# vineety/sparse_matrix_mult

Hardware: AMD Instinct MI355X
Metric: output nnz/sec, CSR x CSR -> CSR SpGEMM (first-touch order, float64) (higher is better)
Workload: dtype f64

## Files before the change

### sparse_matrix_mult_amd/csrc/smm_api.hip

```cpp
#include "smm_kernels.hpp"
#include "smm_slab.hpp"
#include "smm_ring.hpp"
#include "smm_triple_sparse.hpp"
#include "smm_masked.hpp"
#include "smm_spmm.hpp"
#include "smm_kron.hpp"
#include "smm_cg.hpp"
#include "smm_slq.hpp"
#include "smm_sddmm.hpp"
#include "smm_taper.hpp"
#include "smm_interp.hpp"
#include "../../include/smm_hip.h"

#include <sys/mman.h>
#include <unistd.h>

#include <algorithm>
#include <atomic>
#include <cmath>
#include <condition_variable>
#include <cstdarg>
#include <cstdio>
#include <cstring>
#include <map>
// ... 82 lines not shown
    hipEvent_t cg_ev[2] = {nullptr, nullptr};
    int exact_checked = 0;
    int check = 0;
    int inject_alloc_nth = 0;
    bool inject_alloc_hard = false;
    int64_t alloc_retries = 0;
    unsigned *d_flags = nullptr;
    unsigned *d_err = nullptr;
    std::recursive_mutex mu;
};
#define CTX_LOCK(c) std::lock_guard<std::recursive_mutex> ctx_lock_((c)->mu)

static void pool_flush(smm_ctx *c)
{
    for (auto &b : c->pool) (void)hipFree(b.p);
    c->pool.clear();
}
static hipError_t dev_malloc(smm_ctx *c, void **p, size_t bytes)
{
    bool fail_first = false, fail_both = false;
    if (c->inject_alloc_nth > 0 && --c->inject_alloc_nth == 0) { fail_first = true; fail_both = c->inject_alloc_hard; }
    hipError_t e = fail_first ? hipErrorOutOfMemory : hipMalloc(p, bytes);
    if (e == hipSuccess) return e;
    (void)hipGetLastError();
    pool_flush(c);
    ++c->alloc_retries;
    e = fail_both ? hipErrorOutOfMemory : hipMalloc(p, bytes);
    if (e != hipSuccess) { (void)hipGetLastError(); *p = nullptr; }
    return e;
}

static int pool_alloc(smm_ctx *c, size_t bytes, void **out)
{
    if (bytes == 0) bytes = 16;
    bytes = (bytes + 255) & ~(size_t)255;
    int best = -1;
    for (int i = 0; i < (int)c->pool.size(); ++i)
        if (c->pool[i].bytes >= bytes && c->pool[i].bytes <= bytes + bytes / 4 + (1 << 20) &&
            (best < 0 || c->pool[i].bytes < c->pool[best].bytes))
            best = i;
    if (best >= 0) {
        *out = c->pool[best].p;
        c->live[*out] = c->pool[best].bytes;
        c->pool.erase(c->pool.begin() + best);
        return SMM_OK;
    }
    void *p = nullptr;
    hipError_t e = dev_malloc(c, &p, bytes);
    if (e != hipSuccess) return fail(SMM_ERR_ALLOC, "hipMalloc of %zu bytes failed: %s", bytes, hipGetErrorString(e));
    c->live[p] = bytes;
    *out = p;
    return SMM_OK;
}
static void pool_free(smm_ctx *c, void *p)
{
    if (!p) return;
    auto it = c->live.find(p);
    if (it == c->live.end()) return;
    c->pool.push_back({p, it->second});
    c->live.erase(it);
}
template <typename T> static int pool_get(smm_ctx *c, size_t count, T **out)
{
    void *p = nullptr;
    int rc = pool_alloc(c, count * sizeof(T), &p);
    *out = (T *)p;
    return rc;
}

template <typename T> struct PoolBuf {
    smm_ctx *c;
    T *p = nullptr;
    explicit PoolBuf(smm_ctx *ctx) : c(ctx) {}
    PoolBuf(PoolBuf &&o) noexcept : c(o.c), p(o.release()) {}
    PoolBuf &operator=(PoolBuf &&o) noexcept { if (this != &o) { reset(); c = o.c; p = o.release(); } return *this; }
    ~PoolBuf() { reset(); }
    int alloc(size_t count) { reset(); return pool_get(c, count, &p); }
    void reset() { pool_free(c, p); p = nullptr; }
    T *release() { T *q = p; p = nullptr; return q; }
    operator T *() const { return p; }
};
template <typename T> struct DevBuf {
    T *p = nullptr;
    int64_t bytes = 0;
    DevBuf() = default;
    DevBuf(DevBuf &&o) noexcept : p(o.p), bytes(o.bytes) { o.p = nullptr; o.bytes = 0; }
    DevBuf &operator=(DevBuf &&o) noexcept { if (this != &o) { reset(); std::swap(p, o.p); std::swap(bytes, o.bytes); } return *this; }
    ~DevBuf() { reset(); }
    hipError_t alloc(smm_ctx *c, size_t count)
    {
        reset();
        const hipError_t e = dev_malloc(c, (void **)&p, count * sizeof(T));
        if (e == hipSuccess) bytes = (int64_t)(count * sizeof(T));
        return e;
    }
    void reset() { if (p) (void)hipFree(p); p = nullptr; bytes = 0; }
    operator T *() const { return p; }
};
template <auto Destroy> struct Destroyer {
    template <typename T> void operator()(T *x) const { Destroy(x); }
};

struct LaunchTimer {
    smm_ctx *c; const char *name; hipEvent_t t0 = nullptr, t1 = nullptr;
    LaunchTimer(smm_ctx *ctx, const char *n) : c(ctx), name(n)
    {
// ... 917 lines not shown
    if (lds > 64 * 1024)
        HIPCHK(hipFuncSetAttribute((const void *)kern, hipFuncAttributeMaxDynamicSharedMemorySize, (int)lds));
    int64_t grid = (int64_t)args.m * args.nct;
    if (grid > 0x7fffffff) return fail(SMM_ERR_INVALID, "too many (row, tile) units for one launch");
    args.unit_counter = nullptr; args.n_units = (unsigned)grid;
    const bool persist = c->numeric_persist == 2 || (c->numeric_persist == 1 && OUT == OUT_SPARSE);
    if (persist && grid > c->n_cu) {
        const int64_t per_cu = std::max<int64_t>(1, std::min<int64_t>(32 / NW, (int64_t)(160 * 1024) / (int64_t)(lds + 64)));
        args.unit_counter = (unsigned *)((char *)c->d_flags + 220);
        HIPCHK(hipMemsetAsync(args.unit_counter, 0, sizeof(unsigned), c->stream));
        grid = std::min<int64_t>(grid, per_cu * c->n_cu);
    }
#ifdef SMM_STAMPS
    PoolBuf<unsigned long long> d_st(c);
    CHK(d_st.alloc(4));
    (void)hipMemsetAsync(d_st, 0, 32, c->stream);
    args.stamps = d_st;
#endif
    LAUNCH(c, SCR ? "smm_emit" : OUT == OUT_SPARSE ? "smm_numeric" : "smm_numeric_dense", kern, grid, NW * 64, lds, args);
    hipError_t e = hipGetLastError();
#ifdef SMM_STAMPS
    {
        unsigned long long h[4];
        (void)hipMemcpyAsync(h, d_st, 32, hipMemcpyDeviceToHost, c->stream);
        (void)hipStreamSynchronize(c->stream);
        const double tot = (double)(h[0] + h[1] + h[2]);
        fprintf(stderr, "[SMM_STAMPS] units=%lld NW=%d wc=%d nct=%d exact=%d  init %.1f%%  accumulate %.1f%%  epilogue %.1f%%  (sum %.3g cycles)\n",
                (long long)grid, NW, args.wc, args.nct, (int)EXACT, 100 * h[0] / tot, 100 * h[1] / tot, 100 * h[2] / tot, tot);
        d_st.reset();
    }
#endif
    if (e != hipSuccess) return fail(SMM_ERR_HIP, "smm_numeric launch: %s", hipGetErrorString(e));
    return SMM_OK;
}
template <int OUT>
static int launch_numeric(smm_ctx *c, NumericArgs &args, bool sym, int nw, bool exact)
{
    if (args.m <= 0) return SMM_OK;
    args.dummy_idx = (const int *)((const char *)c->d_flags + 64);
    args.dummy_val = (const double *)((const char *)c->d_flags + 128);
    args.err = c->d_err;
#define SMM_CASE(S, N, X) \
    if (sym == S && nw == N && exact == X) return launch_numeric_t<OUT, S, N, X>(c, args);
    SMM_CASE(false, 1, true) SMM_CASE(true, 1, true) SMM_CASE(false, 2, true) SMM_CASE(true, 2, true)
    SMM_CASE(false, 4, true) SMM_CASE(true, 4, true) SMM_CASE(false, 8, true) SMM_CASE(true, 8, true)
    SMM_CASE(false, 16, true) SMM_CASE(true, 16, true)
    SMM_CASE(false, 4, false) SMM_CASE(true, 4, false) SMM_CASE(false, 8, false) SMM_CASE(true, 8, false)
    SMM_CASE(false, 16, false) SMM_CASE(true, 16, false)
#undef SMM_CASE
    return fail(SMM_ERR_INVALID, "unsupported numeric configuration");
}

constexpr size_t LIST_SLACK = (size_t)1 << 17;
#ifndef SMM_CCS_UNROLL
#define SMM_CCS_UNROLL 8
#endif
using ccs_kernel_t = decltype(&smm_symbolic_ccs<false, SMM_CCS_UNROLL>);
static ccs_kernel_t ccs_kernel(bool sym, bool dr, bool batch)
{
#define CCS_K(S, D, B) smm_symbolic_ccs<S, SMM_CCS_UNROLL, D, B>
    if (batch) return dr ? (sym ? CCS_K(true, true, 16) : CCS_K(false, true, 16)) : (sym ? CCS_K(true, false, 16) : CCS_K(false, false, 16));
    return dr ? (sym ? CCS_K(true, true, 1) : CCS_K(false, true, 1)) : (sym ? CCS_K(true, false, 1) : CCS_K(false, false, 1));
#undef CCS_K
}
struct SlabGeom { int ws, n_slabs, rw; };
constexpr int SLAB_NW = 8;
struct smm_plan {
    smm_ctx *ctx = nullptr;
    smm_csr *a = nullptr, *b = nullptr;
    int flags = 0;
    int64_t row_offset = 0;
    int64_t m = 0, ncols = 0, nnz = 0;
    bool b_sorted = true;
    Geom g{};
    int64_t *d_ub_off = nullptr;
    void *d_tmp = nullptr;
    bool list16 = false;
    unsigned *d_P = nullptr;
    unsigned *d_runs = nullptr;
    int2 *d_tail = nullptr;
    int n_slabs = 1, tps = 0, ws = 0;
    int *d_scnt = nullptr;
    unsigned *d_dst0 = nullptr;
    uint2 *d_runs2 = nullptr;
    unsigned char *d_tflag = nullptr;
    const int *seg = nullptr;
    const short *loc = nullptr;
    smm_csr::PackView pack{0, 0, nullptr, nullptr, 0, 0};
    bool use_slab = false;
    SlabGeom sg{};
    smm_csr::SlabView slab{0, 0, nullptr, nullptr, nullptr};
    int *d_rowcnt = nullptr;
    int64_t total_cap = 0;
    int *d_lists = nullptr;
    int n_bin[8] = {0, 0, 0, 0, 0, 0, 0, 0};
    int64_t *d_cptr = nullptr;
};

extern "C" void smm_plan_destroy(smm_plan *p)
{
    if (!p) return;
    smm_ctx *c = p->ctx;
    CTX_LOCK(c);
    (void)hipSetDevice(c->device);
    (void)hipStreamSynchronize(c->stream);
    pool_free(c, p->d_ub_off); pool_free(c, p->d_tmp); pool_free(c, p->d_P); pool_free(c, p->d_runs);
// ... 576 lines not shown
static int sym_slab_walk(smm_ctx *c, smm_plan *p, SymRows &r)
{
    r.slists.reset();
    r.prod.reset();
    smm_csr *a = p->a, *b = p->b;
    const int64_t m = p->m;
    const int ws_cap = c->sym_max_ws > 0 ? c->sym_max_ws : CCS_MAX_WS;
    int tps = std::max(1, std::min(8, ws_cap / p->g.wc));
    if (c->sym_max_ws == 0)
        while (tps > 1 && (160 * 1024) / ((((tps * p->g.wc + 31) / 32) + WAVE) * 4) < 28) --tps;
    p->tps = tps; p->ws = tps * p->g.wc; p->n_slabs = (p->g.nct + tps - 1) / tps;
    p->list16 = true;
    const int ns = p->n_slabs;
    smm_csr::CcsView cc{};
    CHK(ensure_ccs(c, b, p->ws, ns, &cc));
    const int *sseg = nullptr;
    CHK(ensure_seg(c, b, tiles_geom(ns, p->ws), &sseg));
    PoolBuf<int64_t> ubs(c);
    CHK(ubs.alloc((size_t)ns * m));
    pool_free(c, p->d_ub_off); p->d_ub_off = nullptr;
    CHK(pool_get(c, (size_t)ns * m + 1, &p->d_ub_off));
    LAUNCH(c, "smm_row_work", smm_ccs_row_work, (int)std::min<int64_t>((m + 3) / 4, 16384), 256, 0, (int)m, ns, p->ws, (int)p->ncols,
           (int)b->rows, p->row_offset, (p->flags & SMM_SYMMETRIC) ? 1 : 0, a->ptr, a->idx, sseg, ubs.p);
    CHK(scan_launch<int64_t>(c, (int64_t)ns * m, ubs, p->d_ub_off));
    HIPCHK(hipMemcpyAsync(&p->total_cap, p->d_ub_off + (int64_t)ns * m, sizeof(int64_t), hipMemcpyDeviceToHost, c->stream));
    HIPCHK(hipStreamSynchronize(c->stream));
    ubs.reset();
    CHK(pool_alloc(c, ((size_t)std::max<int64_t>(p->total_cap, 1) + LIST_SLACK) * 2, &p->d_tmp));
    CHK(pool_get(c, (size_t)a->nnz * ns, &p->d_P));
    CHK(pool_get(c, (size_t)ns * m, &p->d_scnt));
    CHK(pool_get(c, (size_t)m, &p->d_rowcnt));
    int *d_unitctr = (int *)((char *)c->d_flags + 208);
    HIPCHK(hipMemsetAsync(d_unitctr, 0, sizeof(int), c->stream));
    if ((int64_t)ns * m >= INT32_MAX) return fail(SMM_ERR_INVALID, "too many (slab, row) units");
    CHK(launch_ccs(c, p, cc, (int64_t)ns * m, ns, nullptr, nullptr, p->d_scnt, d_unitctr));
    LAUNCH(c, "smm_slab_rowcnt", smm_slab_rowcnt, std::min<int64_t>((m + 255) / 256, 4096), 256, 0, (int)m, ns, (const int *)p->d_scnt,
           p->d_rowcnt);
    CHK(scan_launch<int>(c, m, p->d_rowcnt, p->d_cptr));
    HIPCHK(hipMemcpyAsync(&p->nnz, p->d_cptr + m, sizeof(int64_t), hipMemcpyDeviceToHost, c->stream));
    HIPCHK(hipStreamSynchronize(c->stream));
    LAUNCH_CHECK();
    if (p->nnz > 0) CHK(bin_c_rows(c, p, BinSpec{2, {0, 0, 0, 0, 0, 0}, 3, 4}, nullptr));
    if (p->n_bin[2] > 0) {
        if (p->flags & SMM_EXACT) {
            CHK(ensure_seg(c, b, p->g, &p->seg));
            CHK(ensure_loc(c, b, p->g, &p->loc));
        } else {
            CHK(ensure_pack(c, b, p->g, PACK_FMT_16, &p->pack));
        }
        CHK(pool_get(c, (size_t)a->nnz, &p->d_dst0));
        CHK(pool_get(c, (size_t)a->nnz * p->g.nct, &p->d_runs2));
        CHK(pool_get(c, (size_t)m * p->g.nct, &p->d_tflag));
        const int nd = p->n_bin[2];
        LAUNCH(c, "smm_runs", smm_runs_slab, std::min<int64_t>((nd + 3) / 4, 65536), 256, 0, nd, (int)m, ns, tps, p->g.nct, p->g.wc,
               (int64_t)a->nnz, (const int *)(p->d_lists + 2 * m), a->ptr, (const int64_t *)p->d_ub_off, (const int *)p->d_scnt,
               (const unsigned *)p->d_P, (const unsigned short *)p->d_tmp, p->d_dst0, p->d_runs2, p->d_tflag, c->d_err);
        LAUNCH_CHECK();
    }
    return SMM_OK;
}

static int sym_row_walk(smm_ctx *c, smm_plan *p, SymRows &r)
{
    smm_csr *a = p->a, *b = p->b;
    const int64_t m = p->m;
    const bool sym = (p->flags & SMM_SYMMETRIC) != 0;
    const bool safe = r.safe;
    p->list16 = c->narrow_idx && p->ncols < 65535 && b->cols < 65535;
    if (p->list16) CHK(ensure_idx16(c, b));
    p->total_cap = r.total_ub;
    CHK(pool_alloc(c, ((size_t)std::max<int64_t>(r.total_ub, 1) + std::max<size_t>(LIST_SLACK, (size_t)p->ncols)) * (p->list16 ? 2 : 4),
                   &p->d_tmp));
    CHK(pool_get(c, (size_t)a->nnz, &p->d_P));
    CHK(pool_get(c, (size_t)m, &p->d_rowcnt));
    if (r.binned) HIPCHK(hipMemsetAsync(p->d_rowcnt, 0, (size_t)m * sizeof(int), c->stream));
    int *d_rowctr = (int *)((char *)c->d_flags + 288);
    HIPCHK(hipMemsetAsync(d_rowctr, 0, 8 * sizeof(int), c->stream));
    int *d_scounts = (int *)((char *)c->d_flags + 256);
    const int *d_slists = r.slists;
    for (int tc = 0; tc < 2; ++tc) {
        const int bin = tc == 0 ? SB_TINY : SB_TINY2;
        const int nt = r.sbin[bin];
        if (nt == 0) continue;
        const int per_wg = tc == 0 ? 16 : 8;
        const int tgrid = (int)std::min<int64_t>(((int64_t)nt + per_wg - 1) / per_wg, (int64_t)c->n_cu * 32);
        const int *rows3 = d_slists + (size_t)bin * m;
#define TINY_CASE(S, IT, G)                                                                                                      \
        LAUNCH(c, "smm_symbolic_tiny", (smm_symbolic_tiny<S, IT, G>), tgrid, 256, 0, nt, rows3, p->row_offset, a->ptr, a->idx,     \
               b->ptr, b->idx, (const int64_t *)p->d_ub_off, (IT *)p->d_tmp, p->d_P, p->d_rowcnt, c->d_err);
#define TINY_G_CASE(S, IT) if (tc == 0) { TINY_CASE(S, IT, TINY_G) } else { TINY_CASE(S, IT, TINY_G2) }
        if (p->list16) { if (sym) { TINY_G_CASE(true, unsigned short) } else { TINY_G_CASE(false, unsigned short) } }
        else           { if (sym) { TINY_G_CASE(true, int) } else { TINY_G_CASE(false, int) } }
#undef TINY_G_CASE
#undef TINY_CASE
        LAUNCH_CHECK();
    }
    for (int cls = 0; cls < NHC; ++cls) {
        if (r.hmax1 == 0 || r.sbin[cls] == 0) continue;
        const int hs = HS[cls];
        const int hgrid = (int)std::min<int64_t>((r.sbin[cls] + 3) / 4, (int64_t)c->n_cu * 16);
        if (sym) CHK((launch_symbolic_t<true, false, MARK_LDS_HASH>(c, p, hs, nullptr, hgrid, 4, d_slists + (size_t)cls * m, d_scounts + cls, d_rowctr + cls)));
        else     CHK((launch_symbolic_t<false, false, MARK_LDS_HASH>(c, p, hs, nullptr, hgrid, 4, d_slists + (size_t)cls * m, d_scounts + cls, d_rowctr + cls)));
    }
    const int bm_words = (int)((p->ncols + 31) / 32);
    const size_t bm_bytes = (size_t)(bm_words + 1) * sizeof(unsigned);
    const bool ldsbm = bm_bytes <= 128 * 1024;
// ... 6 lines not shown
    PoolBuf<unsigned> gbm(c);
    const bool use_ccs = c->sym_ccs && p->list16 && !safe && p->ncols <= CCS_MAX_WS && nbm > 0;
    if (use_ccs) {
        smm_csr::CcsView cc{};
        CHK(ensure_ccs(c, b, (int)p->ncols, 1, &cc));
        CHK(launch_ccs(c, p, cc, nbm, 1, bm_rows, bm_count, p->d_rowcnt, d_rowctr + SB_REST));
    } else if (nbm > 0) {
        int sgrid = (int)std::min<int64_t>((nbm + wpb - 1) / wpb, (int64_t)c->n_cu * 8 * (4 / wpb));
        if (!ldsbm) CHK(gbm.alloc((size_t)sgrid * wpb * (bm_words + 1)));
        const int mark = ldsbm ? MARK_LDS_BITMAP : MARK_GLOBAL_BITMAP;
        const int rbatch = nbm >= (int64_t)64 * sgrid * wpb && nbm < INT32_MAX - (1 << 24) ? 16 : 1;
#define SYM_CASE(S, F, L) if (sym == S && safe == F && mark == L && !deep) CHK((launch_symbolic_t<S, F, L>(c, p, bm_words, gbm, sgrid, wpb, bm_rows, bm_count, d_rowctr + SB_REST, rbatch)));
        SYM_CASE(false, false, MARK_LDS_BITMAP) SYM_CASE(false, true, MARK_LDS_BITMAP) SYM_CASE(true, false, MARK_LDS_BITMAP)
        SYM_CASE(true, true, MARK_LDS_BITMAP) SYM_CASE(false, false, MARK_GLOBAL_BITMAP) SYM_CASE(false, true, MARK_GLOBAL_BITMAP)
        SYM_CASE(true, false, MARK_GLOBAL_BITMAP) SYM_CASE(true, true, MARK_GLOBAL_BITMAP)
#define SYM_DEEP(S, L) if (sym == S && mark == L && deep) CHK((launch_symbolic_t<S, false, L, 32>(c, p, bm_words, gbm, sgrid, wpb, bm_rows, bm_count, d_rowctr + SB_REST, rbatch)));
        SYM_DEEP(false, MARK_LDS_BITMAP) SYM_DEEP(true, MARK_LDS_BITMAP) SYM_DEEP(false, MARK_GLOBAL_BITMAP) SYM_DEEP(true, MARK_GLOBAL_BITMAP)
#undef SYM_DEEP
#undef SYM_CASE
    }
    CHK(scan_launch<int>(c, m, p->d_rowcnt, p->d_cptr));
    HIPCHK(hipMemcpyAsync(&p->nnz, p->d_cptr + m, sizeof(int64_t), hipMemcpyDeviceToHost, c->stream));
    HIPCHK(hipStreamSynchronize(c->stream));
    LAUNCH_CHECK();
    gbm.reset();
    r.slists.reset();
    return SMM_OK;
}

static int sym_runs(smm_ctx *c, smm_plan *p, SymRows &r)
{
    smm_csr *a = p->a, *b = p->b;
    const int64_t m = p->m;
    if (p->nnz > 0) CHK(bin_c_rows(c, p, BinSpec{2, {c->hash_small, c->hash_medium, 0, 0, 0, 0}, 3, 4}, r.prod));
    r.prod.reset();
    if (!p->b_sorted || p->n_bin[2] == 0) return SMM_OK;
    const double est_products = (double)a->nnz * ((double)b->nnz / (double)std::max<int64_t>(b->rows, 1)) * ((double)p->n_bin[2] / (double)m);
    p->use_slab = slab_geometry(c, b, p->ncols, &p->sg) &&
                  slab_pays(c, a, p->sg, (double)p->n_bin[2] * (double)p->ncols, est_products, (double)p->nnz,
                            (double)b->nnz / (double)std::max<int64_t>(b->rows, 1), (double)p->ncols);
    if (p->use_slab) CHK(ensure_slab(c, b, p->sg, &p->slab));
    if (p->use_slab && c->slab_mode == 2) {  }
    else if (p->flags & SMM_EXACT) {
        CHK(ensure_seg(c, b, p->g, &p->seg));
        CHK(ensure_loc(c, b, p->g, &p->loc));
    } else {
        CHK(ensure_pack(c, b, p->g, p->use_slab ? PACK_FMT_16 : PACK_FMT_12, &p->pack));
    }
    CHK(pool_get(c, (size_t)a->nnz * (p->g.nct + 1), &p->d_runs));
    CHK(pool_get(c, (size_t)m, &p->d_tail));
    const int nd = p->n_bin[2];
    const int rgrid = (int)std::min<int64_t>((nd + 3) / 4, 65536);
    const int tail_min = (p->flags & SMM_EXACT) ? TAIL_MIN_EXACT : TAIL_MIN_DEFAULT;
    if (p->list16)
        LAUNCH(c, "smm_runs", smm_runs<unsigned short>, rgrid, 256, 0, nd, p->g.nct, p->g.wc, (const int *)(p->d_lists + 2 * m), a->ptr,
               p->d_ub_off, p->d_rowcnt, p->d_P, (const unsigned short *)p->d_tmp, p->d_runs, p->d_tail, c->d_err, tail_min);
    else
        LAUNCH(c, "smm_runs", smm_runs<int>, rgrid, 256, 0, nd, p->g.nct, p->g.wc, (const int *)(p->d_lists + 2 * m), a->ptr,
               p->d_ub_off, p->d_rowcnt, p->d_P, (const int *)p->d_tmp, p->d_runs, p->d_tail, c->d_err, tail_min);
    LAUNCH_CHECK();
    return SMM_OK;
}

extern "C" int smm_spgemm_symbolic(smm_ctx *c, smm_csr *a, smm_csr *b, int flags, int64_t a_row_offset,
                                   smm_plan **plan, int64_t *nnz_out)
{
    if (!plan) return fail(SMM_ERR_INVALID, "plan is NULL");
    *plan = nullptr;
    if (!c) return fail(SMM_ERR_INVALID, "ctx is NULL");
    CTX_LOCK(c);
    CHK(check_pair(c, a, b));
    if (a_row_offset < 0) return fail(SMM_ERR_INVALID, "negative a_row_offset");
    CHK(exact_guard(c, flags));
    PlanPtr p(new smm_plan());
    p->ctx = c; p->a = a; p->b = b; p->flags = flags; p->row_offset = a_row_offset;
    p->m = a->rows; p->ncols = b->cols;
    p->b_sorted = !(b->vflags & CSR_UNSORTED);
    p->g = make_geom(c, p->ncols, b, (flags & SMM_EXACT) != 0);
    CHK(pool_get(c, (size_t)p->m + 1, &p->d_cptr));
    if (p->m == 0 || a->nnz == 0 || b->nnz == 0 || p->ncols == 0) {
        HIPCHK(hipMemsetAsync(p->d_cptr, 0, (p->m + 1) * sizeof(int64_t), c->stream));
    } else {
        SymRows r(c);
        CHK(sym_row_work(c, p.get(), r));
        if (use_slab_walk(c, p.get(), r)) {
            CHK(sym_slab_walk(c, p.get(), r));
        } else {
            CHK(sym_row_walk(c, p.get(), r));
            CHK(sym_runs(c, p.get(), r));
        }
        if (c->check) CHK(plan_check(c, p.get()));
    }
    if (nnz_out) *nnz_out = p->nnz;
    *plan = p.release();
    return SMM_OK;
}

extern "C" int smm_spgemm_numeric(smm_ctx *c, smm_plan *p, int64_t *d_c_indptr, int32_t *d_c_indices, double *d_c_data)
{
    if (!c || !p || p->ctx != c) return fail(SMM_ERR_INVALID, "bad plan/context");
    if (!d_c_indptr) return fail(SMM_ERR_INVALID, "d_c_indptr is NULL");
    HIPCHK(hipSetDevice(c->device));
    CTX_LOCK(c);
    const int64_t m = p->m;
    HIPCHK(hipMemcpyAsync(d_c_indptr, p->d_cptr, (m + 1) * sizeof(int64_t), hipMemcpyDeviceToDevice, c->stream));
    if (p->nnz == 0) return SMM_OK;
// ... 2084 lines not shown
```

### sparse_matrix_mult_amd/csrc/smm_kernels.hpp

```cpp
#pragma once
#include <hip/hip_runtime.h>
#include <stdint.h>
#include <type_traits>

namespace smm {

constexpr int WAVE = 64;
enum { OUT_SPARSE = 0, OUT_DENSE = 1 };

enum { CSR_BAD = 1, CSR_UNSORTED = 2, CSR_HAS_EQUAL = 4 };

enum {
    PLAN_ERR_RUNS = 1,
    PLAN_ERR_TAIL = 2,
    PLAN_ERR_RUNS2 = 4,
    PLAN_ERR_P = 8,
    PLAN_ERR_HASH = 16,
    PLAN_ERR_CAP = 32,
    PLAN_ERR_COUNT = 64,
    PLAN_ERR_LIST = 128,
    PLAN_ERR_PIECE = 512,
};
#ifndef SMM_CLAMPS
#define SMM_CLAMPS 1
#endif
__device__ __forceinline__ void plan_err(unsigned *err, unsigned bit, int row) {
    atomicOr(err, bit);
    atomicMin(err + 1, (unsigned)row);
}

__device__ __forceinline__ int lane_id() { return (int)(threadIdx.x & 63u); }

__device__ __forceinline__ int rl(int v, int l) { return __builtin_amdgcn_readlane(v, l); }
__device__ __forceinline__ unsigned rl(unsigned v, int l) {
    return (unsigned)__builtin_amdgcn_readlane((int)v, l);
}
__device__ __forceinline__ double rl(double v, int l) {
    int lo = __double2loint(v), hi = __double2hiint(v);
    return __hiloint2double(__builtin_amdgcn_readlane(hi, l), __builtin_amdgcn_readlane(lo, l));
}
__device__ __forceinline__ int mbcnt(unsigned long long mask) {
    return (int)__builtin_amdgcn_mbcnt_hi((unsigned)(mask >> 32),
                                          __builtin_amdgcn_mbcnt_lo((unsigned)mask, 0u));
}
__device__ __forceinline__ void wave_sync() {
    __builtin_amdgcn_fence(__ATOMIC_RELEASE, "wavefront");
    __builtin_amdgcn_wave_barrier();
    __builtin_amdgcn_fence(__ATOMIC_ACQUIRE, "wavefront");
}
__device__ __forceinline__ void load_masked(int &v, const int *idx, unsigned long long mask, int lane4) {
    asm volatile("s_mov_b64 exec, %3\n\t"
                 "global_load_dword %0, %1, %2\n\t"
                 "s_mov_b64 exec, -1"
                 : "+v"(v)
// ... 943 lines not shown
                                const unsigned packed = (unsigned)c[u] | ((unsigned)ch[u] << 16);
                                asm volatile("s_mov_b64 exec, %4\n\t"
                                             "global_store_short %0, %2, %3\n\t"
                                             "s_mov_b64 exec, %5\n\t"
                                             "global_store_short_d16_hi %1, %2, %3\n\t"
                                             "s_mov_b64 exec, -1"
                                             :: "v"(off_lo), "v"(off_hi), "v"(packed), "s"(out), "s"(ml), "s"(mh) : "memory");
                            }
#else
                            if (nl_) out[at] = (unsigned short)c[u];
                            if (nh_) out[at + (nl_ ? 1u : 0u)] = (unsigned short)ch[u];
#endif
                            n += __popcll(ml) + __popcll(mh);
                        }
                    }
                    const int tl = excl - tg;
                    const bool has = nch > 0 && tl >= 0 && tl < G;
                    const int pv = __shfl(nrec, has ? tl : 0);
                    if (has) myP = (unsigned)pv;
                }
                {
                    unsigned v = myP;
#pragma unroll
                    for (int o = 1; o < WAVE; o <<= 1) {
                        const unsigned y = __shfl_down(v, o);
                        if (lane + o < WAVE && y < v) v = y;
                    }
                    if (v == 0xffffffffu) v = (unsigned)n;
                    if (lane < nb) Ps[jb + lane] = v;
                }
                cs = cs_n; ce = ce_n; r_n = r_nn;
            }
        }
        if (lane == 0) cnt[(size_t)s * m + row] = n;
#if SMM_CCS_ASM_STORES
        asm volatile("s_waitcnt vmcnt(0)" ::: "memory");
#endif
        if (n >= bm_words) {
            for (int w = lane; w < bm_words; w += WAVE) bm[w] = 0;
        } else {
            for (int s2 = lane; s2 < n; s2 += WAVE) bm[out[s2] >> 5] = 0;
        }
      }
    }
}

#ifndef SMM_TAIL_MIN_DEFAULT
#define SMM_TAIL_MIN_DEFAULT 32
#endif
#ifndef SMM_TAIL_MIN_EXACT
#define SMM_TAIL_MIN_EXACT 64
#endif
constexpr int TAIL_MIN_DEFAULT = SMM_TAIL_MIN_DEFAULT, TAIL_MIN_EXACT = SMM_TAIL_MIN_EXACT;
constexpr int RUNS_WIN = 2048;
template <typename LT>
__global__ __launch_bounds__(256) void smm_runs(int m, int nct, int wc, const int *__restrict__ rowlist,
                                                const int *__restrict__ a_ptr,
                                                const int64_t *__restrict__ ub_off,
                                                const int *__restrict__ rowcnt,
                                                const unsigned *__restrict__ P,
                                                const LT *__restrict__ tmp_idx,
                                                unsigned *__restrict__ runs, int2 *__restrict__ tail, unsigned *__restrict__ err,
                                                int tail_min)
{
    __shared__ int win_all[4][RUNS_WIN];
    constexpr int NV = RUNS_WIN / WAVE;
    const int lane = lane_id();
    const int wpb = blockDim.x / WAVE;
    int *win = win_all[threadIdx.x >> 6];
    for (int ri = blockIdx.x * wpb + (threadIdx.x >> 6); ri < m; ri += gridDim.x * wpb) {
        const int row = rowlist ? rowlist[ri] : ri;
        const int a0 = a_ptr[row], a1 = a_ptr[row + 1];
        const LT *__restrict__ list = tmp_idx + ub_off[row];
        const unsigned total = (unsigned)rowcnt[row];
        int e_last = a0 - 1;
        for (int eb = a0; eb < a1; eb += WAVE) {
            const int e = eb + lane;
            if (e < a1) {
                const unsigned q0 = P[e], q1 = e + 1 < a1 ? P[e + 1] : total;
                if (q1 - q0 >= (unsigned)tail_min) e_last = e;
            }
        }
        for (int o = 32; o > 0; o >>= 1) { const int y = __shfl_xor(e_last, o); e_last = y > e_last ? y : e_last; }
        const int e0 = e_last + 1;
        if (lane == 0) tail[row] = make_int2(e0, (int)(e0 < a1 ? P[e0] : total));
        int v[NV];
        auto fetch = [&](unsigned wb) {
#pragma unroll
            for (int u = 0; u < NV; ++u) {
                const unsigned i = wb + u * WAVE + lane;
                v[u] = (int)list[i < total ? i : (total ? total - 1 : 0)];
            }
        };
        unsigned cur = 0xffffffffu;
        if (total) fetch(0);
        for (int eb = a0; eb < e0; eb += WAVE) {
            const int e = eb + lane;
            const bool valid = e < e0;
            unsigned p0 = valid ? P[e] : total;
            unsigned p1 = (valid && e + 1 < a1) ? P[e + 1] : total;
            if (p0 > total || p1 > total || p1 < p0) {
                plan_err(err, PLAN_ERR_P, row);
                p0 = p0 < total ? p0 : total;
                p1 = p1 < p0 ? p0 : (p1 < total ? p1 : total);
            }
            unsigned *r = runs + (size_t)(valid ? e : e0 - 1) * (nct + 1);
            int tcur = 1;
            if (valid) {
                r[0] = p0; r[nct] = p1;
                if (p0 == p1) { for (; tcur < nct; ++tcur) r[tcur] = p0; }
            } else {
                tcur = nct;
            }
            const unsigned reg_lo = rl(p0, 0), reg_hi = rl(p1, WAVE - 1);
            for (unsigned wb = reg_lo - reg_lo % RUNS_WIN; wb < reg_hi; wb += RUNS_WIN) {
                const unsigned we = wb + RUNS_WIN < total ? wb + RUNS_WIN : total;
                if (wb != cur) {
                    wave_sync();
#pragma unroll
                    for (int u = 0; u < NV; ++u) win[u * WAVE + lane] = v[u];
                    cur = wb;
                    if (we < total) fetch(we);
                    wave_sync();
                }
                unsigned lo = p0 > wb ? p0 : wb;
                const unsigned hiw = p1 < we ? p1 : we;
                if (lo < hiw) {
                    while (tcur < nct) {
                        const int bound = tcur * wc;
                        unsigned l = lo, h = hiw;
                        while (l < h) {
                            const unsigned mid = l + ((h - l) >> 1);
                            if (win[mid - wb] < bound) l = mid + 1; else h = mid;
                        }
                        if (l < hiw) { r[tcur] = l; lo = l; ++tcur; }
                        else if (p1 <= we) { r[tcur] = p1; lo = hiw; ++tcur; }
                        else break;
                    }
                }
            }
        }
    }
}

__global__ __launch_bounds__(256) void smm_slab_rowcnt(int m, int n_slabs, const int *__restrict__ scnt, int *__restrict__ rowcnt)
{
    for (int row = blockIdx.x * blockDim.x + threadIdx.x; row < m; row += gridDim.x * blockDim.x) {
        int t = 0;
        for (int s = 0; s < n_slabs; ++s) t += scnt[(size_t)s * m + row];
        rowcnt[row] = t;
    }
}

__global__ __launch_bounds__(256) void smm_runs_slab(int nrows, int m, int n_slabs, int tps, int nct, int wc, int64_t nnzA,
                                                     const int *__restrict__ rowlist, const int *__restrict__ a_ptr,
                                                     const int64_t *__restrict__ list_off, const int *__restrict__ scnt,
                                                     const unsigned *__restrict__ P, const unsigned short *__restrict__ tmp,
                                                     unsigned *__restrict__ dst0, uint2 *__restrict__ runs2,
                                                     unsigned char *__restrict__ tflag, unsigned *__restrict__ err)
{
    __shared__ int win_all[4][RUNS_WIN];
    constexpr int NV = RUNS_WIN / WAVE;
    constexpr int TPS_MAX = 8;
    const int lane = lane_id();
    const int wpb = blockDim.x / WAVE;
    int *win = win_all[threadIdx.x >> 6];
    for (int ri = blockIdx.x * wpb + (threadIdx.x >> 6); ri < nrows; ri += gridDim.x * wpb) {
        const int row = rowlist ? rowlist[ri] : ri;
        const int a0 = a_ptr[row], a1 = a_ptr[row + 1];
        auto cnt_of = [&](int s, int e) -> unsigned {
            const unsigned *Ps = P + (size_t)s * nnzA;
            const unsigned q1 = e + 1 < a1 ? Ps[e + 1] : (unsigned)scnt[(size_t)s * m + row];
            const unsigned q0 = Ps[e];
            return q1 >= q0 ? q1 - q0 : 0u;
        };
        unsigned carry = 0;
        for (int eb = a0; eb < a1; eb += WAVE) {
            const int e = eb + lane;
            int C = 0;
            if (e < a1)
                for (int s = 0; s < n_slabs; ++s) C += (int)cnt_of(s, e);
            const int incl = wave_scan_incl(C);
            if (e < a1) dst0[e] = carry + (unsigned)(incl - C);
            carry += (unsigned)rl(incl, WAVE - 1);
        }
        for (int s = 0; s < n_slabs; ++s) {
            const int t0 = s * tps;
            const int tsl = (nct - t0) < tps ? (nct - t0) : tps;
            const unsigned short *__restrict__ list = tmp + list_off[(size_t)s * m + row];
            const unsigned total = (unsigned)scnt[(size_t)s * m + row];
            const unsigned *__restrict__ Ps = P + (size_t)s * nnzA;
            int v[NV];
            auto fetch = [&](unsigned wb) {
#pragma unroll
                for (int u = 0; u < NV; ++u) {
                    const unsigned i = wb + u * WAVE + lane;
                    v[u] = (int)list[i < total ? i : (total ? total - 1 : 0)];
                }
            };
            unsigned cur = 0xffffffffu;
            if (total) fetch(0);
            for (int eb = a0; eb < a1; eb += WAVE) {
                const int e = eb + lane;
                const bool valid = e < a1;
                unsigned p0 = valid ? Ps[e] : total;
                unsigned p1 = (valid && e + 1 < a1) ? Ps[e + 1] : total;
                if (p0 > total || p1 > total || p1 < p0) {
                    plan_err(err, PLAN_ERR_P, row);
                    p0 = p0 < total ? p0 : total;
                    p1 = p1 < p0 ? p0 : (p1 < total ? p1 : total);
                }
                uint2 *r = runs2 + (size_t)t0 * nnzA + (valid ? e : a1 - 1);
                int tcur = 1;
                if (valid) {
                    r[0].x = p0;
                    if (p0 == p1) { for (; tcur < tsl; ++tcur) r[(size_t)tcur * nnzA].x = p0; }
                } else {
                    tcur = tsl;
                }
                const unsigned reg_lo = rl(p0, 0), reg_hi = rl(p1, WAVE - 1);
                for (unsigned wb = reg_lo - reg_lo % RUNS_WIN; wb < reg_hi; wb += RUNS_WIN) {
                    const unsigned we = wb + RUNS_WIN < total ? wb + RUNS_WIN : total;
                    if (wb != cur) {
                        wave_sync();
#pragma unroll
                        for (int u = 0; u < NV; ++u) win[u * WAVE + lane] = v[u];
                        cur = wb;
                        if (we < total) fetch(we);
                        wave_sync();
                    }
                    unsigned lo = p0 > wb ? p0 : wb;
                    const unsigned hiw = p1 < we ? p1 : we;
                    if (lo < hiw) {
                        while (tcur < tsl) {
                            const int bound = tcur * wc;
                            unsigned l = lo, h = hiw;
                            while (l < h) {
                                const unsigned mid = l + ((h - l) >> 1);
                                if (win[mid - wb] < bound) l = mid + 1; else h = mid;
                            }
                            if (l < hiw) { r[(size_t)tcur * nnzA].x = l; lo = l; ++tcur; }
                            else if (p1 <= we) { r[(size_t)tcur * nnzA].x = p1; lo = hiw; ++tcur; }
                            else break;
                        }
                    }
                }
            }
            __threadfence_block();
            unsigned any = 0;
            for (int eb = a0; eb < a1; eb += WAVE) {
                const int e = eb + lane;
                if (e >= a1) continue;
                unsigned p0 = Ps[e];
                unsigned p1 = e + 1 < a1 ? Ps[e + 1] : total;
                p0 = p0 < total ? p0 : total;
                p1 = p1 < p0 ? p0 : (p1 < total ? p1 : total);
                unsigned base = dst0[e];
                for (int sp = 0; sp < s; ++sp) base += cnt_of(sp, e);
                uint2 *r = runs2 + (size_t)t0 * nnzA + e;
                unsigned st = r[0].x;
                for (int tt = 0; tt < tsl; ++tt) {
                    const unsigned en = tt + 1 < tsl ? r[(size_t)(tt + 1) * nnzA].x : p1;
                    r[(size_t)tt * nnzA] = make_uint2(st | ((en - st) << 16), base + (st - p0));
                    any |= (en != st ? 1u : 0u) << tt;
                    st = en;
                }
            }
            for (int tt = 0; tt < tsl && tt < TPS_MAX; ++tt) {
                const bool some = __ballot((any >> tt) & 1u) != 0ull;
                if (lane == 0) tflag[(size_t)(t0 + tt) * m + row] = some ? 1 : 0;
            }
        }
    }
}

struct NumericArgs {
    int m, ncols, nct, wc, wf, n_ft;
    int64_t row_offset;
    const int *a_ptr, *a_idx; const double *a_val;
    const int *b_idx; const double *b_val;
    const short *b_loc;
    const int2 *tdesc; const double *tpay; int rowsB;
    int piece_epl;
    int piece_fmt;
    int tstride;
    const unsigned short *tlen16;
    const int *seg;
    int kmax;
    const int *dummy_idx;
    const double *dummy_val;
    const int64_t *c_ptr; int *c_idx; double *c_val;
    const int64_t *ub_off; const void *tmp_idx;
// ... 1701 lines not shown
```

Measured before the change: 83.64 billion.

## Vectorize run-window list loads and stage run outputs through LDS for coalescing

The smm_runs and smm_runs_slab kernels now load the sorted column list window with 16-byte vector loads, aligning window starts to the list's base offset and keeping the window in its native element width (16-bit or 32-bit) in shared memory instead of widening it to int. When the tile count is small, smm_runs stages per-entry run boundaries in LDS and writes them back coalesced instead of issuing strided scattered stores. Host-side checks assert the list buffer is 16-byte aligned and that a window fits the allocation slack, because the vector loads may read past the end of a row's list.

```diff
diff --git a/sparse_matrix_mult_amd/csrc/smm_api.hip b/sparse_matrix_mult_amd/csrc/smm_api.hip
--- a/sparse_matrix_mult_amd/csrc/smm_api.hip
+++ b/sparse_matrix_mult_amd/csrc/smm_api.hip
@@ -158,6 +158,11 @@
     *out = p;
     return SMM_OK;
 }
+static int list_base_aligned(const void *d_tmp)
+{
+    if (((uintptr_t)d_tmp & 15) != 0) return fail(SMM_ERR_INTERNAL, "the list buffer %p is not 16-byte aligned", d_tmp);
+    return SMM_OK;
+}
 static void pool_free(smm_ctx *c, void *p)
 {
     if (!p) return;
@@ -1181,6 +1186,7 @@
 }
 
 constexpr size_t LIST_SLACK = (size_t)1 << 17;
+static_assert((size_t)RUNS_WIN <= LIST_SLACK && (size_t)RUNS_WIN16 <= LIST_SLACK, "a staged window must fit the slack behind the lists");
 #ifndef SMM_CCS_UNROLL
 #define SMM_CCS_UNROLL 8
 #endif
@@ -1863,6 +1869,7 @@
         CHK(pool_get(c, (size_t)a->nnz * p->g.nct, &p->d_runs2));
         CHK(pool_get(c, (size_t)m * p->g.nct, &p->d_tflag));
         const int nd = p->n_bin[2];
+        CHK(list_base_aligned(p->d_tmp));
         LAUNCH(c, "smm_runs", smm_runs_slab, std::min<int64_t>((nd + 3) / 4, 65536), 256, 0, nd, (int)m, ns, tps, p->g.nct, p->g.wc,
                (int64_t)a->nnz, (const int *)(p->d_lists + 2 * m), a->ptr, (const int64_t *)p->d_ub_off, (const int *)p->d_scnt,
                (const unsigned *)p->d_P, (const unsigned short *)p->d_tmp, p->d_dst0, p->d_runs2, p->d_tflag, c->d_err);
@@ -1975,6 +1982,7 @@
     const int nd = p->n_bin[2];
     const int rgrid = (int)std::min<int64_t>((nd + 3) / 4, 65536);
     const int tail_min = (p->flags & SMM_EXACT) ? TAIL_MIN_EXACT : TAIL_MIN_DEFAULT;
+    CHK(list_base_aligned(p->d_tmp));
     if (p->list16)
         LAUNCH(c, "smm_runs", smm_runs<unsigned short>, rgrid, 256, 0, nd, p->g.nct, p->g.wc, (const int *)(p->d_lists + 2 * m), a->ptr,
                p->d_ub_off, p->d_rowcnt, p->d_P, (const unsigned short *)p->d_tmp, p->d_runs, p->d_tail, c->d_err, tail_min);
diff --git a/sparse_matrix_mult_amd/csrc/smm_kernels.hpp b/sparse_matrix_mult_amd/csrc/smm_kernels.hpp
--- a/sparse_matrix_mult_amd/csrc/smm_kernels.hpp
+++ b/sparse_matrix_mult_amd/csrc/smm_kernels.hpp
@@ -1,5 +1,6 @@
 #pragma once
 #include <hip/hip_runtime.h>
+#include <limits.h>
 #include <stdint.h>
 #include <type_traits>
 
@@ -1049,7 +1050,39 @@
 #define SMM_TAIL_MIN_EXACT 64
 #endif
 constexpr int TAIL_MIN_DEFAULT = SMM_TAIL_MIN_DEFAULT, TAIL_MIN_EXACT = SMM_TAIL_MIN_EXACT;
+#ifndef SMM_RUNS_WIN16
+#define SMM_RUNS_WIN16 2048
+#endif
 constexpr int RUNS_WIN = 2048;
+constexpr int RUNS_WIN16 = SMM_RUNS_WIN16;
+typedef unsigned runs_v4 __attribute__((ext_vector_type(4)));
+template <typename LT> struct RunsWindow {
+    static constexpr int WIN = sizeof(LT) == 2 ? RUNS_WIN16 : RUNS_WIN;
+    static constexpr int EPV = 16 / (int)sizeof(LT);
+    static constexpr int NV = WIN / EPV / WAVE;
+    static constexpr int ALIGN = 128 / (int)sizeof(LT);
+    static_assert(NV >= 1 && NV * EPV * WAVE == WIN && (WIN & (WIN - 1)) == 0 && ALIGN <= WIN, "window geometry");
+    runs_v4 v[NV];
+    __device__ __forceinline__ void fetch(const LT *__restrict__ list, int wb, int total, int lane) {
+        const runs_v4 *__restrict__ src = reinterpret_cast<const runs_v4 *>(list + wb) + lane;
+        const int left = total - wb - lane * EPV;
+#pragma unroll
+        for (int u = 0; u < NV; ++u)
+            if (u * WAVE * EPV < left) v[u] = src[u * WAVE];
+    }
+    __device__ __forceinline__ void store(LT *win, int lane) const {
+        runs_v4 *dst = reinterpret_cast<runs_v4 *>(win) + lane;
+#pragma unroll
+        for (int u = 0; u < NV; ++u) dst[u * WAVE] = v[u];
+    }
+    static __device__ __forceinline__ int start_of(unsigned p, int sh) {
+        return (int)((p + (unsigned)sh) & ~(unsigned)(WIN - 1)) - sh;
+    }
+};
+__device__ __forceinline__ int64_t rl64(int64_t v) {
+    return (int64_t)(((unsigned long long)rl((unsigned)((unsigned long long)v >> 32), 0) << 32) | rl((unsigned)v, 0));
+}
+constexpr int RUNS_STAGE = 8;
 template <typename LT>
 __global__ __launch_bounds__(256) void smm_runs(int m, int nct, int wc, const int *__restrict__ rowlist,
                                                 const int *__restrict__ a_ptr,
@@ -1060,16 +1093,22 @@
                                                 unsigned *__restrict__ runs, int2 *__restrict__ tail, unsigned *__restrict__ err,
                                                 int tail_min)
 {
-    __shared__ int win_all[4][RUNS_WIN];
-    constexpr int NV = RUNS_WIN / WAVE;
+    using Win = RunsWindow<LT>;
+    constexpr int WIN = Win::WIN;
+    __shared__ __attribute__((aligned(16))) LT win_all[4][WIN];
+    __shared__ unsigned stage_all[4][WAVE * RUNS_STAGE];
     const int lane = lane_id();
     const int wpb = blockDim.x / WAVE;
-    int *win = win_all[threadIdx.x >> 6];
+    LT *win = win_all[threadIdx.x >> 6];
+    unsigned *stg = stage_all[threadIdx.x >> 6] + lane * (nct + 1);
+    const bool staged = nct + 1 <= RUNS_STAGE;
     for (int ri = blockIdx.x * wpb + (threadIdx.x >> 6); ri < m; ri += gridDim.x * wpb) {
         const int row = rowlist ? rowlist[ri] : ri;
         const int a0 = a_ptr[row], a1 = a_ptr[row + 1];
-        const LT *__restrict__ list = tmp_idx + ub_off[row];
-        const unsigned total = (unsigned)rowcnt[row];
+        const int64_t off = rl64(ub_off[row]);
+        const LT *__restrict__ list = tmp_idx + off;
+        const int sh = (int)(off & (Win::ALIGN - 1));
+        const unsigned total = rl((unsigned)rowcnt[row], 0);
         int e_last = a0 - 1;
         for (int eb = a0; eb < a1; eb += WAVE) {
             const int e = eb + lane;
@@ -1080,61 +1119,63 @@
         }
         for (int o = 32; o > 0; o >>= 1) { const int y = __shfl_xor(e_last, o); e_last = y > e_last ? y : e_last; }
         const int e0 = e_last + 1;
-        if (lane == 0) tail[row] = make_int2(e0, (int)(e0 < a1 ? P[e0] : total));
-        int v[NV];
-        auto fetch = [&](unsigned wb) {
-#pragma unroll
-            for (int u = 0; u < NV; ++u) {
-                const unsigned i = wb + u * WAVE + lane;
-                v[u] = (int)list[i < total ? i : (total ? total - 1 : 0)];
-            }
-        };
-        unsigned cur = 0xffffffffu;
-        if (total) fetch(0);
+        const unsigned tail_at = e0 < a1 ? P[e0] : total;
+        if (lane == 0) tail[row] = make_int2(e0, (int)tail_at);
+        Win w;
+        int cur = INT_MIN;
+        if (total && e0 > a0) w.fetch(list, -sh, (int)total, lane);
         for (int eb = a0; eb < e0; eb += WAVE) {
             const int e = eb + lane;
             const bool valid = e < e0;
-            unsigned p0 = valid ? P[e] : total;
-            unsigned p1 = (valid && e + 1 < a1) ? P[e + 1] : total;
+            unsigned p0 = valid ? P[e] : tail_at;
+            unsigned p1 = valid ? (e + 1 < a1 ? P[e + 1] : total) : tail_at;
             if (p0 > total || p1 > total || p1 < p0) {
                 plan_err(err, PLAN_ERR_P, row);
                 p0 = p0 < total ? p0 : total;
                 p1 = p1 < p0 ? p0 : (p1 < total ? p1 : total);
             }
             unsigned *r = runs + (size_t)(valid ? e : e0 - 1) * (nct + 1);
+            auto put = [&](int t, unsigned x) { if (staged) stg[t] = x; else r[t] = x; };
             int tcur = 1;
             if (valid) {
-                r[0] = p0; r[nct] = p1;
-                if (p0 == p1) { for (; tcur < nct; ++tcur) r[tcur] = p0; }
+                put(0, p0); put(nct, p1);
+                if (p0 == p1) { for (; tcur < nct; ++tcur) put(tcur, p0); }
             } else {
                 tcur = nct;
             }
             const unsigned reg_lo = rl(p0, 0), reg_hi = rl(p1, WAVE - 1);
-            for (unsigned wb = reg_lo - reg_lo % RUNS_WIN; wb < reg_hi; wb += RUNS_WIN) {
-                const unsigned we = wb + RUNS_WIN < total ? wb + RUNS_WIN : total;
+            for (int wb = Win::start_of(reg_lo, sh); (wb > 0 ? wb : 0) < (int)reg_hi; wb += WIN) {
+                const int we = wb + WIN < (int)total ? wb + WIN : (int)total;
                 if (wb != cur) {
                     wave_sync();
-#pragma unroll
-                    for (int u = 0; u < NV; ++u) win[u * WAVE + lane] = v[u];
+                    w.store(win, lane);
                     cur = wb;
-                    if (we < total) fetch(we);
+                    if (we < (int)total) w.fetch(list, we, (int)total, lane);
                     wave_sync();
                 }
-                unsigned lo = p0 > wb ? p0 : wb;
-                const unsigned hiw = p1 < we ? p1 : we;
+                unsigned lo = (int)p0 > wb ? p0 : (unsigned)wb;
+                const unsigned hiw = p1 < (unsigned)we ? p1 : (unsigned)we;
                 if (lo < hiw) {
                     while (tcur < nct) {
                         const int bound = tcur * wc;
                         unsigned l = lo, h = hiw;
                         while (l < h) {
                             const unsigned mid = l + ((h - l) >> 1);
-                            if (win[mid - wb] < bound) l = mid + 1; else h = mid;
+                            if ((int)win[(int)mid - wb] < bound) l = mid + 1; else h = mid;
                         }
-                        if (l < hiw) { r[tcur] = l; lo = l; ++tcur; }
-                        else if (p1 <= we) { r[tcur] = p1; lo = hiw; ++tcur; }
+                        if (l < hiw) { put(tcur, l); lo = l; ++tcur; }
+                        else if (p1 <= we) { put(tcur, p1); lo = hiw; ++tcur; }
                         else break;
                     }
                 }
+            }
+            if (staged) {
+                wave_sync();
+                const int nst = e0 - eb < WAVE ? e0 - eb : WAVE;
+                unsigned *dst = runs + (size_t)eb * (nct + 1);
+                const unsigned *src = stage_all[threadIdx.x >> 6];
+                for (int j = lane; j < nst * (nct + 1); j += WAVE) dst[j] = src[j];
+                wave_sync();
             }
         }
     }
@@ -1156,12 +1197,13 @@
                                                      unsigned *__restrict__ dst0, uint2 *__restrict__ runs2,
                                                      unsigned char *__restrict__ tflag, unsigned *__restrict__ err)
 {
-    __shared__ int win_all[4][RUNS_WIN];
-    constexpr int NV = RUNS_WIN / WAVE;
+    using Win = RunsWindow<unsigned short>;
+    constexpr int WIN = Win::WIN;
+    __shared__ __attribute__((aligned(16))) unsigned short win_all[4][WIN];
     constexpr int TPS_MAX = 8;
     const int lane = lane_id();
     const int wpb = blockDim.x / WAVE;
-    int *win = win_all[threadIdx.x >> 6];
+    unsigned short *win = win_all[threadIdx.x >> 6];
     for (int ri = blockIdx.x * wpb + (threadIdx.x >> 6); ri < nrows; ri += gridDim.x * wpb) {
         const int row = rowlist ? rowlist[ri] : ri;
         const int a0 = a_ptr[row], a1 = a_ptr[row + 1];
@@ -1184,19 +1226,14 @@
         for (int s = 0; s < n_slabs; ++s) {
             const int t0 = s * tps;
             const int tsl = (nct - t0) < tps ? (nct - t0) : tps;
-            const unsigned short *__restrict__ list = tmp + list_off[(size_t)s * m + row];
-            const unsigned total = (unsigned)scnt[(size_t)s * m + row];
+            const int64_t off = rl64(list_off[(size_t)s * m + row]);
+            const unsigned short *__restrict__ list = tmp + off;
+            const int sh = (int)(off & (Win::ALIGN - 1));
+            const unsigned total = rl((unsigned)scnt[(size_t)s * m + row], 0);
             const unsigned *__restrict__ Ps = P + (size_t)s * nnzA;
-            int v[NV];
-            auto fetch = [&](unsigned wb) {
-#pragma unroll
-                for (int u = 0; u < NV; ++u) {
-                    const unsigned i = wb + u * WAVE + lane;
-                    v[u] = (int)list[i < total ? i : (total ? total - 1 : 0)];
-                }
-            };
-            unsigned cur = 0xffffffffu;
-            if (total) fetch(0);
+            Win w;
+            int cur = INT_MIN;
+            if (total) w.fetch(list, -sh, (int)total, lane);
             for (int eb = a0; eb < a1; eb += WAVE) {
                 const int e = eb + lane;
                 const bool valid = e < a1;
@@ -1216,25 +1253,24 @@
                     tcur = tsl;
                 }
                 const unsigned reg_lo = rl(p0, 0), reg_hi = rl(p1, WAVE - 1);
-                for (unsigned wb = reg_lo - reg_lo % RUNS_WIN; wb < reg_hi; wb += RUNS_WIN) {
-                    const unsigned we = wb + RUNS_WIN < total ? wb + RUNS_WIN : total;
+                for (int wb = Win::start_of(reg_lo, sh); (wb > 0 ? wb : 0) < (int)reg_hi; wb += WIN) {
+                    const int we = wb + WIN < (int)total ? wb + WIN : (int)total;
                     if (wb != cur) {
                         wave_sync();
-#pragma unroll
-                        for (int u = 0; u < NV; ++u) win[u * WAVE + lane] = v[u];
+                        w.store(win, lane);
                         cur = wb;
-                        if (we < total) fetch(we);
+                        if (we < (int)total) w.fetch(list, we, (int)total, lane);
                         wave_sync();
                     }
-                    unsigned lo = p0 > wb ? p0 : wb;
-                    const unsigned hiw = p1 < we ? p1 : we;
+                    unsigned lo = (int)p0 > wb ? p0 : (unsigned)wb;
+                    const unsigned hiw = p1 < (unsigned)we ? p1 : (unsigned)we;
                     if (lo < hiw) {
                         while (tcur < tsl) {
                             const int bound = tcur * wc;
                             unsigned l = lo, h = hiw;
                             while (l < h) {
                                 const unsigned mid = l + ((h - l) >> 1);
-                                if (win[mid - wb] < bound) l = mid + 1; else h = mid;
+                                if ((int)win[(int)mid - wb] < bound) l = mid + 1; else h = mid;
                             }
                             if (l < hiw) { r[(size_t)tcur * nnzA].x = l; lo = l; ++tcur; }
                             else if (p1 <= we) { r[(size_t)tcur * nnzA].x = p1; lo = hiw; ++tcur; }
```

Measured after the change: 83.93 billion, median of 6. No clear change (+0.3%).
